# RenderKit/embree

Hardware: NVIDIA H100
Metric: Mrays/s incoherent diffuse-bounce, 10M-triangle scene (higher is better)
Workload: dtype f32

## Files before the change

### embree_b200/csrc/rtcore_shim.cpp

```cpp
#include <cuda_runtime.h>
#include <math.h>
#include <stdio.h>
#include <stdlib.h>
#include <string.h>

#include <algorithm>
#include <atomic>
#include <map>
#include <mutex>
#include <stdexcept>
#include <string>
#include <unordered_map>
#include <vector>

#include "../../include/embree4_b200.h"
#include "interp.cuh"
#include "rtk_device.h"

namespace {

struct ApiError {
  RTCError code;
  std::string msg;
};
// ... 567 lines not shown
void commit_scene(SceneImpl* s) {
  std::lock_guard<std::mutex> lk(s->commitMutex);
  std::vector<GeometryImpl*> geoms;
  {
    std::lock_guard<std::mutex> lg(s->geomMutex);
    if (!s->isModified()) return;
    geoms = s->geoms;
  }
  for (GeometryImpl* g : geoms)
    if (g && g->enabled && g->state == GeomState::MODIFIED) fail(RTC_ERROR_INVALID_OPERATION, "geometry not committed");
  if (s->progFn && !s->progFn(s->progPtr, 0.0)) fail(RTC_ERROR_CANCELLED, "progress monitor forced termination");
  s->dev->use();
  release_buffers(s->deviceBuffers);
  release_buffers(s->residentBuffers);
  s->residentCurves.clear();
  s->free_interp();
  const TwoLevelChoice twoLevel = choose_two_level(s, geoms);
  if (twoLevel.chosen) commit_two_level(s, geoms);
  else commit_single(s, geoms, twoLevel.possible);
}

struct ThreadCtx {
  int gpu = -1;
  cudaStream_t stream = nullptr;
  static constexpr size_t kStagingBytes = 16384;
  char* staging = nullptr;
  ~ThreadCtx() {
    if (staging) cudaFreeHost(staging);
    if (stream) cudaStreamDestroy(stream);
  }
  void ensure(int g) {
    if (gpu == g && stream) return;
    if (staging) { cudaFreeHost(staging); staging = nullptr; }
    if (stream) { cudaStreamDestroy(stream); stream = nullptr; }
    cudaSetDevice(g);
    cuda_check(cudaStreamCreateWithFlags(&stream, cudaStreamNonBlocking), "cudaStreamCreate");
    cuda_check(cudaHostAlloc(reinterpret_cast<void**>(&staging), kStagingBytes, cudaHostAllocMapped), "cudaHostAlloc");
    gpu = g;
  }
};
thread_local ThreadCtx t_ctx;

struct QueryArgs {
  uint32_t instID = RTC_INVALID_GEOMETRY_ID, instPrimID = RTC_INVALID_GEOMETRY_ID;
  RTCFilterFunctionN filter = nullptr;
  bool enforce = false;
  RTCRayQueryContext* ctx = nullptr;
};
template <typename Args>
QueryArgs read_args(const Args* a) {
  QueryArgs q;
  if (!a) return q;
  q.filter = a->filter;
  q.enforce = (a->flags & RTC_RAY_QUERY_FLAG_INVOKE_ARGUMENT_FILTER) != 0;
  q.ctx = a->context;
  if (a->context) { q.instID = a->context->instID[0]; q.instPrimID = a->context->instPrimID[0]; }
  return q;
}

bool filters_apply(SceneImpl* s, const QueryArgs& q, int occluded) {
  if (!q.filter && g_filterGeoms.load(std::memory_order_relaxed) == 0) return false;
  auto applies = [&](const GeometryImpl* g) {
    if (occluded ? g->occludedFilter != nullptr : g->intersectFilter != nullptr) return true;
    return q.filter && (q.enforce || g->argFilterEnabled);
  };
  std::lock_guard<std::mutex> lg(s->geomMutex);
  for (GeometryImpl* g : s->geoms) {
    if (!g || !g->enabled) continue;
    if (g->type != RTC_GEOMETRY_TYPE_INSTANCE) { if (applies(g)) return true; continue; }
    if (!g->instScene) continue;
    std::lock_guard<std::mutex> lc(g->instScene->geomMutex);
    for (GeometryImpl* cg : g->instScene->geoms)
      if (cg && cg->enabled && cg->type != RTC_GEOMETRY_TYPE_INSTANCE && applies(cg)) return true;
  }
  return false;
}

rtk::TraceParams make_params(SceneImpl* s, void* rays, const int* valid, unsigned long long n, uint32_t instID,
                             uint32_t instPrimID) {
  rtk::TraceParams p;
  p.nodes = s->gpu.nodes; p.tris = s->gpu.tris; p.root_valid = s->gpu.root_valid; p.robust = s->gpu.robust;
  p.descs = s->gpu.general ? s->gpu.d_descs : nullptr;
  p.curves = s->gpu.curves;
  p.top_nodes = s->gpu.levels.size() > 3 ? s->gpu.levels[3] : s->gpu.num_nodes;
  p.rays = rays; p.valid = valid; p.n = n; p.instID = instID; p.instPrimID = instPrimID;
  p.stat = s->statCounters ? s->gpu.d_stat : nullptr;
  return p;
}

void require_committed(SceneImpl* s) {
  if (!s->everCommitted) fail(RTC_ERROR_INVALID_OPERATION, "scene not committed");
}

void trace_one(SceneImpl* s, void* rec, size_t recBytes, const int* valid, int K, int occluded, uint32_t instID,
               uint32_t instPrimID) {
  require_committed(s);
  if (!s->gpu.root_valid) return;
  t_ctx.ensure(s->dev->gpu);
  cudaSetDevice(s->dev->gpu);
  memcpy(t_ctx.staging, rec, recBytes);
  int* sv = reinterpret_cast<int*>(t_ctx.staging + 1408);
  if (K > 1) memcpy(sv, valid, 4 * K);
  rtk::TraceParams p = make_params(s, t_ctx.staging, K > 1 ? sv : nullptr, (unsigned long long)K, instID, instPrimID);
  cuda_check((cudaError_t)rtk::launch_trace(p, occluded, K, t_ctx.stream), "trace launch");
  cuda_check(cudaStreamSynchronize(t_ctx.stream), "trace");
  memcpy(rec, t_ctx.staging, recBytes);
}

void trace_device(SceneImpl* s, void* d_rays, const int* d_valid, int K, size_t M, int occluded, uint32_t instID,
                  uint32_t instPrimID, cudaStream_t st, bool timeit, void* compact_out = nullptr) {
  require_committed(s);
  if (!s->gpu.root_valid || M == 0) return;
  cudaSetDevice(s->dev->gpu);
  rtk::TraceParams p = make_params(s, d_rays, d_valid, (unsigned long long)M * K, instID, instPrimID);
  p.compact_out = compact_out;
  if (timeit) {
    if (!s->ev0) { cudaEventCreate(&s->ev0); cudaEventCreate(&s->ev1); }
    cudaEventRecord(s->ev0, st);
  }
  cuda_check((cudaError_t)rtk::launch_trace(p, occluded, K, st), "trace launch");
  if (timeit) cudaEventRecord(s->ev1, st);
}

void trace_gather(SceneImpl* s, void* d_rays, size_t M, uint32_t instID, uint32_t instPrimID, cudaStream_t st, void* compact_out) {
  require_committed(s);
  if (M == 0) return;
  if (reinterpret_cast<uintptr_t>(compact_out) & 31) fail(RTC_ERROR_INVALID_ARGUMENT, "compact_out must be 32-byte aligned (one sector per record)");
  cudaSetDevice(s->dev->gpu);
  if (!s->ev0) { cudaEventCreate(&s->ev0); cudaEventCreate(&s->ev1); }
  cudaEventRecord(s->ev0, st);
  rtk::TraceParams p = make_params(s, d_rays, nullptr, (unsigned long long)M, instID, instPrimID);
  p.compact_out = compact_out;
  if (rtk::tuning().gather_mode == 1) {
    static thread_local struct Stage { int gpu = -1; void* p = nullptr; size_t cap = 0; ~Stage() { if (p) cudaFree(p); } } t_stage;
    if (t_stage.gpu != s->dev->gpu || t_stage.cap < M * 32) {
      if (t_stage.p) { cudaSetDevice(t_stage.gpu); cudaFree(t_stage.p); cudaSetDevice(s->dev->gpu); }
      t_stage.p = nullptr; t_stage.cap = 0; t_stage.gpu = s->dev->gpu;
      cuda_check(cudaMalloc(&t_stage.p, M * 32), "cudaMalloc(gather staging)");
      t_stage.cap = M * 32;
    }
    p.stage = t_stage.p;
  }
  cuda_check((cudaError_t)rtk::launch_trace(p, 0, 1, st), "trace launch");
  cudaEventRecord(s->ev1, st);
}

static int g_host_chunk_log2 = 20, g_host_streams = 3;
static int g_host_d2h_partial = 0;

struct HostPipe {
  int gpu = -1;
  static constexpr int kStreams = 6;
  cudaStream_t st[kStreams] = {};
  char* buf[kStreams] = {};
  int* vbuf[kStreams] = {};
  size_t cap = 0, vcap = 0;
  ~HostPipe() { reset(); }
  void reset() {
    for (int i = 0; i < kStreams; ++i) {
      if (buf[i]) cudaFree(buf[i]);
      if (vbuf[i]) cudaFree(vbuf[i]);
      if (st[i]) cudaStreamDestroy(st[i]);
      buf[i] = nullptr; vbuf[i] = nullptr; st[i] = nullptr;
    }
    cap = vcap = 0; gpu = -1;
  }
  void ensure(int g, size_t bytes, size_t vbytes) {
// ... 850 lines not shown
  scene_layout(g, &lay);
  s->dev->use();
  if (nodes && lay.num_nodes) cuda_check(cudaMemcpy(nodes, g.nodes, (size_t)lay.num_nodes * sizeof(rtk::Node8), cudaMemcpyDeviceToHost), "copy nodes");
  if (records && lay.num_records) cuda_check(cudaMemcpy(records, g.tris, (size_t)lay.num_records * sizeof(rtk::TriRec), cudaMemcpyDeviceToHost), "copy records");
  if (descs && lay.num_descs) {
    std::vector<rtk::GeomDesc> d(lay.num_descs);
    cuda_check(cudaMemcpy(d.data(), g.d_descs, d.size() * sizeof(rtk::GeomDesc), cudaMemcpyDeviceToHost), "copy descriptors");
    unsigned first = 0;
    for (size_t i = 0; i < d.size(); ++i) {
      RTCB200DescInfo& o = descs[i];
      o.geomID = d[i].geomID; o.instID = d[i].instID; o.kind = d[i].kind; o.first = first; o.count = d[i].ntris;
      o.is_quad = d[i].is_quad; o.tess = d[i].tess; o.basis = d[i].basis; o.hermite = d[i].hermite;
      memcpy(o.xfm, d[i].xfm, sizeof o.xfm);
      first += d[i].ntris;
    }
  }
  if (levels) for (unsigned l = 0; l < lay.num_levels; ++l) levels[l] = g.levels[l];
  if (subs)
    for (unsigned i = 0; i < lay.num_subs; ++i) {
      subs[4 * i] = g.sub_node_off[i]; subs[4 * i + 1] = g.sub_tri_off[i];
      subs[4 * i + 2] = g.sub_nodes[i]; subs[4 * i + 3] = g.sub_tris[i];
    }
  SCENE_END
}
void rtcb200SetSceneStatCounters(RTCScene sc, int enable) { SCENE_BEGIN(sc) S(sc)->statCounters = enable != 0; SCENE_END }
void rtcb200ResetSceneStatCounters(RTCScene sc) { SCENE_BEGIN(sc) if (S(sc)->gpu.d_stat) { S(sc)->dev->use(); cuda_check(cudaMemset(S(sc)->gpu.d_stat, 0, 24), "reset stat counters"); } SCENE_END }
unsigned long long rtcb200GetLaunchCount(void) { return rtk::launch_count(); }

void* rtcb200PeerAlloc(RTCDevice h, size_t bytes) {
  API_BEGIN
  VERIFY_HANDLE(h);
  D(h)->use();
  void* p = nullptr;
  cuda_check(cudaMalloc(&p, bytes ? bytes : 16), "cudaMalloc(peer buffer)");
  return p;
  API_END(D(h))
  return nullptr;
}
void rtcb200PeerFree(RTCDevice h, void* p) { API_BEGIN VERIFY_HANDLE(h); D(h)->use(); if (p) cuda_check(cudaFree(p), "cudaFree(peer buffer)"); API_END(D(h)) }
int rtcb200PeerExport(RTCDevice h, void* p, unsigned char handle[64]) {
  API_BEGIN
  VERIFY_HANDLE(h); VERIFY_HANDLE(p); VERIFY_HANDLE(handle);
  D(h)->use();
  static_assert(sizeof(cudaIpcMemHandle_t) == 64, "IPC handle size");
  cudaIpcMemHandle_t ih;
  cuda_check(cudaIpcGetMemHandle(&ih, p), "cudaIpcGetMemHandle");
  memcpy(handle, &ih, 64);
  return 0;
  API_END(D(h))
  return -1;
}
void* rtcb200PeerImport(RTCDevice h, const unsigned char handle[64]) {
  API_BEGIN
  VERIFY_HANDLE(h); VERIFY_HANDLE(handle);
  D(h)->use();
  cudaIpcMemHandle_t ih;
  memcpy(&ih, handle, 64);
  void* p = nullptr;
  cuda_check(cudaIpcOpenMemHandle(&p, ih, cudaIpcMemLazyEnablePeerAccess), "cudaIpcOpenMemHandle");
  return p;
  API_END(D(h))
  return nullptr;
}
void rtcb200PeerCopy(RTCDevice h, void* dst, const void* src, size_t bytes) {
  API_BEGIN VERIFY_HANDLE(h); D(h)->use(); cuda_check(cudaMemcpy(dst, src, bytes, cudaMemcpyDefault), "cudaMemcpy(peer buffer)"); API_END(D(h))
}
void rtcb200PeerClose(RTCDevice h, void* p) { API_BEGIN VERIFY_HANDLE(h); D(h)->use(); if (p) cuda_check(cudaIpcCloseMemHandle(p), "cudaIpcCloseMemHandle"); API_END(D(h)) }
int rtcb200SetTuning(const char* key, int value) {
  if (!key) return -1;
  rtk::Tuning& t = rtk::tuning();
  if (!strcmp(key, "collapse_policy")) t.collapse_policy = value;
  else if (!strcmp(key, "refill_min")) t.refill_min = value;
  else if (!strcmp(key, "sah_small")) t.sah_small = value;
  else if (!strcmp(key, "c_node")) t.c_node = value;
  else if (!strcmp(key, "c_tri")) t.c_tri = value;
  else if (!strcmp(key, "tri_batch_min")) t.tri_batch_min = value;
  else if (!strcmp(key, "tri_wait_max")) t.tri_wait_max = value;
  else if (!strcmp(key, "curve_batch_min")) t.curve_batch_min = value;
  else if (!strcmp(key, "curve_wait_max")) t.curve_wait_max = value;
  else if (!strcmp(key, "blocks_per_sm")) t.blocks_per_sm = value;
  else if (!strcmp(key, "curve_blocks_per_sm")) t.curve_blocks_per_sm = value;
  else if (!strcmp(key, "point_batch_min")) t.point_batch_min = value;
  else if (!strcmp(key, "point_wait_max")) t.point_wait_max = value;
  else if (!strcmp(key, "use_tma")) t.use_tma = value;
  else if (!strcmp(key, "tri_spread")) t.tri_spread = value != 0;
  else if (!strcmp(key, "tri_spread_occluded")) t.tri_spread_occluded = value != 0;
  else if (!strcmp(key, "gather_mode") && value >= 0 && value <= 1) t.gather_mode = value;
  else if (!strcmp(key, "host_d2h_partial")) g_host_d2h_partial = value != 0;
  else if (!strcmp(key, "host_chunk_log2") && value >= 10 && value <= 26) g_host_chunk_log2 = value;
  else if (!strcmp(key, "host_streams") && value >= 1 && value <= HostPipe::kStreams) g_host_streams = value;
  else return -1;
  return 0;
}
double rtcb200GetLastTraceMs(RTCScene sc) {
  SCENE_BEGIN(sc)
  SceneImpl* s = S(sc);
  if (!s->ev0) return -1.0;
  s->dev->use();
  cuda_check(cudaEventSynchronize(s->ev1), "event sync");
  float ms = 0;
  cuda_check(cudaEventElapsedTime(&ms, s->ev0, s->ev1), "event elapsed");
  return ms;
  SCENE_END
  return -1.0;
}

static void load_transform(RTCFormat format, const float* x, float out[12]) {
  switch ((int)format) {
    case 0x9134: { const float m[12] = {x[0], x[4], x[8], x[1], x[5], x[9], x[2], x[6], x[10], x[3], x[7], x[11]}; memcpy(out, m, sizeof m); break; }
    case 0x9234: memcpy(out, x, 12 * sizeof(float)); break;
    case 0x9244: { const float m[12] = {x[0], x[1], x[2], x[4], x[5], x[6], x[8], x[9], x[10], x[12], x[13], x[14]}; memcpy(out, m, sizeof m); break; }
    default: fail(RTC_ERROR_INVALID_OPERATION, "invalid matrix format");
  }
}
static void store_transform(const float m[12], RTCFormat format, float* x) {
  switch ((int)format) {
    case 0x9134: { const float o[12] = {m[0], m[3], m[6], m[9], m[1], m[4], m[7], m[10], m[2], m[5], m[8], m[11]}; memcpy(x, o, sizeof o); break; }
    case 0x9234: memcpy(x, m, 12 * sizeof(float)); break;
    case 0x9244: { const float o[16] = {m[0], m[1], m[2], 0, m[3], m[4], m[5], 0, m[6], m[7], m[8], 0, m[9], m[10], m[11], 1}; memcpy(x, o, sizeof o); break; }
    default: fail(RTC_ERROR_INVALID_OPERATION, "invalid matrix format");
  }
}
void rtcSetGeometryInstancedScene(RTCGeometry g, RTCScene scene) {
  GEOM_BEGIN(g)
  VERIFY_HANDLE(scene);
  if (G(g)->type != RTC_GEOMETRY_TYPE_INSTANCE) fail(RTC_ERROR_INVALID_OPERATION, "operation not supported for this geometry");
  if (G(g)->dev != S(scene)->dev) fail(RTC_ERROR_INVALID_ARGUMENT, "inputs are from different devices");
  S(scene)->retain();
  if (G(g)->instScene) G(g)->instScene->release();
  G(g)->instScene = S(scene);
  G(g)->update();
  GEOM_END
}
void rtcSetGeometryTransform(RTCGeometry g, unsigned int timeStep, enum RTCFormat format, const void* xfm) {
  GEOM_BEGIN(g)
  VERIFY_HANDLE(xfm);
  if (G(g)->type != RTC_GEOMETRY_TYPE_INSTANCE) fail(RTC_ERROR_INVALID_OPERATION, "operation not supported for this geometry");
  if (timeStep != 0) fail(RTC_ERROR_INVALID_OPERATION, "invalid timestep");
  load_transform(format, static_cast<const float*>(xfm), G(g)->xfm);
  G(g)->update_world2local();
  G(g)->update();
  GEOM_END
}
void rtcGetGeometryTransform(RTCGeometry g, float, enum RTCFormat format, void* xfm) {
  GEOM_BEGIN(g)
  VERIFY_HANDLE(xfm);
  store_transform(G(g)->xfm, format, static_cast<float*>(xfm));
  GEOM_END
}
void rtcGetGeometryTransformEx(RTCGeometry g, unsigned int, float time, enum RTCFormat format, void* xfm) { rtcGetGeometryTransform(g, time, format, xfm); }
void rtcGetGeometryTransformFromScene(RTCScene s, unsigned int id, float time, enum RTCFormat format, void* xfm) {
  SCENE_BEGIN(s)
  if (id >= S(s)->geoms.size() || !S(s)->geoms[id]) fail(RTC_ERROR_INVALID_ARGUMENT, "invalid geometry ID");
  rtcGetGeometryTransform(reinterpret_cast<RTCGeometry>(S(s)->geoms[id]), time, format, xfm);
  SCENE_END
}
void rtcGetGeometryTransformFromTraversable(RTCTraversable t, unsigned int id, float time, enum RTCFormat format, void* xfm) {
  rtcGetGeometryTransformFromScene(reinterpret_cast<RTCScene>(t), id, time, format, xfm);
}

void* rtcGetGeometryBufferDataDevice(RTCGeometry g, enum RTCBufferType type, unsigned int slot) { return rtcGetGeometryBufferData(g, type, slot); }
void rtcSetSharedGeometryBufferHostDevice(RTCGeometry g, enum RTCBufferType type, unsigned int slot, enum RTCFormat format, const void* ptr,
                                          const void* , size_t off, size_t stride, size_t num) {
  rtcSetSharedGeometryBuffer(g, type, slot, format, ptr, off, stride, num);
}
void rtcSetNewGeometryBufferHostDevice(RTCGeometry g, enum RTCBufferType type, unsigned int slot, enum RTCFormat format, size_t stride,
                                       size_t num, void** ptr, void** dptr) {
// ... 81 lines not shown
```

### embree_b200/csrc/rtk_device.h

```cpp
#pragma once
#include <cuda_runtime.h>
#include <stddef.h>
#include <stdint.h>

#include <vector>

#include "rt_core.cuh"

namespace rtk {

enum PrimKind : uint32_t {
  PRIM_TRIANGLE = 0,
  PRIM_ROUND_LINEAR = 1,
  PRIM_FLAT_LINEAR = 2,
  PRIM_FLAT_CUBIC = 3,
  PRIM_ROUND_CUBIC = 4,
  PRIM_SPHERE = 5,
  PRIM_DISC = 6,
  PRIM_ORIENTED_DISC = 7,
};
RT_HD constexpr bool curve_record(uint32_t kind) { return kind >= PRIM_ROUND_LINEAR && kind <= PRIM_ROUND_CUBIC; }
RT_HD constexpr bool point_record(uint32_t kind) { return kind >= PRIM_SPHERE; }

struct GeomDesc {
// ... 2 lines not shown
  uint64_t vstride, istride;
  uint32_t nverts, ntris;
  uint32_t geomID, mask;
  uint32_t has_xfm = 0, instID = 0xFFFFFFFFu, inst_mask = 0xFFFFFFFFu, skip_bounds = 0;
  uint32_t is_quad = 0;
  uint32_t kind = PRIM_TRIANGLE;
  const uint8_t* flags = nullptr;
  uint32_t basis = 0, tess = 4, hermite = 0;
  const float* basis_tab = nullptr;
  const uint8_t* tangents = nullptr;
  uint64_t tstride = 0;
  float xfm[12] = {1, 0, 0, 0, 1, 0, 0, 0, 1, 0, 0, 0};
  float w2l[12] = {1, 0, 0, 0, 1, 0, 0, 0, 1, 0, 0, 0};
};

#if defined(__CUDACC__)
__device__ __forceinline__ void load_cubic_cp(const GeomDesc& g, uint32_t vid, CurveVtx cp[4]) {
  if (g.hermite) {
    const float4 p0 = __ldg(reinterpret_cast<const float4*>(g.verts + (size_t)vid * g.vstride));
    const float4 p1 = __ldg(reinterpret_cast<const float4*>(g.verts + (size_t)(vid + 1) * g.vstride));
    const float4 t0 = __ldg(reinterpret_cast<const float4*>(g.tangents + (size_t)vid * g.tstride));
    const float4 t1 = __ldg(reinterpret_cast<const float4*>(g.tangents + (size_t)(vid + 1) * g.tstride));
    const float k = 1.0f / 3.0f;
    cp[0] = CurveVtx{p0.x, p0.y, p0.z, p0.w};
    cp[1] = CurveVtx{fma_rn(k, t0.x, p0.x), fma_rn(k, t0.y, p0.y), fma_rn(k, t0.z, p0.z), fma_rn(k, t0.w, p0.w)};
    cp[2] = CurveVtx{fma_rn(-k, t1.x, p1.x), fma_rn(-k, t1.y, p1.y), fma_rn(-k, t1.z, p1.z), fma_rn(-k, t1.w, p1.w)};
    cp[3] = CurveVtx{p1.x, p1.y, p1.z, p1.w};
    return;
  }
#pragma unroll
  for (int k = 0; k < 4; ++k) {
    const float4 q = __ldg(reinterpret_cast<const float4*>(g.verts + (size_t)(vid + k) * g.vstride));
    cp[k] = CurveVtx{q.x, q.y, q.z, q.w};
  }
}
#endif

enum BuilderKind : uint32_t { BUILDER_LBVH = 0, BUILDER_SAH = 1 };

struct SceneGPU {
  int device = 0;
  Node8* nodes = nullptr;
  TriRec* tris = nullptr;
  uint32_t num_nodes = 0, num_tris = 0;
  uint32_t root_valid = 0;
  int robust = 0;
  int general = 0;
  int curves = 0;
  GeomDesc* d_descs = nullptr;
  uint32_t num_descs = 0;
  float bounds[6] = {0, 0, 0, 0, 0, 0};
  float api_bounds[6] = {0, 0, 0, 0, 0, 0};
  double build_ms = 0, sah_cost = 0;
  uint32_t builder = 0, max_depth = 0;
  unsigned long long* d_stat = nullptr;
  size_t node_capacity = 0, tri_capacity = 0;
  uint32_t* tri_src = nullptr;
  uint32_t total_prims = 0;
  std::vector<uint32_t> levels;
  std::vector<uint32_t> sub_node_off, sub_tri_off, sub_nodes, sub_tris;
  std::vector<Node8> sub_root;
  std::vector<const void*> sub_id;
  uint32_t top_cap = 0;
  bool is_sub = false;
};

int assemble_scene(SceneGPU& top, SceneGPU* const* subs, int nsubs, const uint8_t* dirty, cudaStream_t stream, char* errmsg);

int build_scene(SceneGPU& s, const GeomDesc* geoms, int ngeoms, BuilderKind kind, cudaStream_t stream, char* errmsg);
int refit_scene(SceneGPU& s, const GeomDesc* geoms, int ngeoms, cudaStream_t stream, char* errmsg);
void free_scene(SceneGPU& s);

struct TraceParams {
  const Node8* nodes;
  const TriRec* tris;
  uint32_t root_valid;
  void* rays;
  const int* valid;
  unsigned long long n;
  uint32_t instID, instPrimID;
  unsigned long long* stat;
  void* compact_out = nullptr;
  void* stage = nullptr;
  int tri_batch_min = 8, tri_wait_max = 4, refill_min = 4, use_prefetch = 1;
  const GeomDesc* descs = nullptr;
  int curves = 0;
  uint32_t top_nodes = 0;
  int robust = 0;
  const uint32_t* excl_off = nullptr;
  const uint32_t* excl_idx = nullptr;
  uint32_t* win = nullptr;
};
int launch_trace(const TraceParams& p, int occluded, int K, cudaStream_t stream);

struct InterpEntry {
  uint32_t kind = 0;
  uint32_t basis = 0;
  uint32_t nprims = 0;
  uint32_t sub = 0;
  const uint8_t* idx = nullptr;
  const uint8_t* data = nullptr;
  const uint8_t* tang = nullptr;
  uint64_t istride = 0, dstride = 0, tstride = 0;
  uint64_t nelems = 0, ntang = 0;
};
struct InterpParams {
  const void* hits;
  unsigned long long M;
  const InterpEntry* table;
  uint32_t nentries;
  uint32_t valueCount;
  float* out[6];
};
int launch_interpolate(const InterpParams& p, cudaStream_t stream);

struct Tuning {
  int collapse_policy = 3;
  int c_node = 100, c_tri = 50;
  int tri_batch_min = 8;
  int tri_wait_max = 4;
  int curve_batch_min = 32, curve_wait_max = 24;
  int point_batch_min = 24, point_wait_max = 16;
  int blocks_per_sm = 8;
  int curve_blocks_per_sm = 6;
  int use_tma = 1;
  int refill_min = 4;
  int gather_mode = 1;
  int tri_spread = 1;
  int tri_spread_occluded = 1;
  int sah_small = 4;
};
Tuning& tuning();

void set_pool_keep_bytes(unsigned long long bytes);
unsigned long long launch_count();
void count_launch(unsigned n = 1);

}
```

### embree_b200/csrc/trace.cu

```cuda
#include <stdio.h>

#include "rtk_device.h"

namespace rtk {

__device__ __forceinline__ void ldg256(const void* p, uint32_t* d) {
  asm volatile("ld.global.nc.v4.b32 {%0,%1,%2,%3}, [%8];\n\t"
               "ld.global.nc.v4.b32 {%4,%5,%6,%7}, [%8+16];"
               : "=r"(d[0]), "=r"(d[1]), "=r"(d[2]), "=r"(d[3]), "=r"(d[4]), "=r"(d[5]), "=r"(d[6]), "=r"(d[7])
               : "l"(p));
}
__device__ __forceinline__ void load_node(const Node8* __restrict__ nodes, uint32_t node_index, NodeW& nw) {
  const char* np = reinterpret_cast<const char*>(nodes) + (size_t)node_index * sizeof(Node8);
  ldg256(np, nw.w); ldg256(np + 32, nw.w + 8); ldg256(np + 64, nw.w + 16);
}

template <int K, bool OCCLUDED>
struct RayIO;

template <bool OCCLUDED>
struct RayIO<1, OCCLUDED> {
  static constexpr int kStride = OCCLUDED ? 48 : 96;
  static constexpr int kRayBytes = kStride;
  static __device__ __forceinline__ void load(const char* base, unsigned long long i, Ray& r) {
    const float4* src = reinterpret_cast<const float4*>(base + i * kStride);
    const float4 a = src[0], b = src[1], c = src[2];
    r.ox = a.x; r.oy = a.y; r.oz = a.z; r.tnear = a.w;
    r.dx = b.x; r.dy = b.y; r.dz = b.z; r.time = b.w;
    r.tfar = c.x; r.mask = __float_as_uint(c.y); r.id = __float_as_uint(c.z); r.flags = __float_as_uint(c.w);
  }
  static __device__ __forceinline__ void store_tfar(const TraceParams& p, unsigned long long i, float tfar) {
    *reinterpret_cast<float*>(static_cast<char*>(p.rays) + i * kStride + 32) = tfar;
  }
  static __device__ __forceinline__ void store_hit(const TraceParams& p, unsigned long long i, const Hit& h, uint32_t instID, uint32_t instPrimID) {
    char* rec = static_cast<char*>(p.rays) + i * kStride;
    *reinterpret_cast<float*>(rec + 32) = h.t;
    float4 a, b;
    a.x = h.ngx; a.y = h.ngy; a.z = h.ngz; a.w = h.u;
    b.x = h.v; b.y = __uint_as_float(h.primID); b.z = __uint_as_float(h.geomID); b.w = __uint_as_float(instID);
    *reinterpret_cast<float4*>(rec + 48) = a;
    *reinterpret_cast<float4*>(rec + 64) = b;
    *reinterpret_cast<uint32_t*>(rec + 80) = instPrimID;
  }
};

template <int K, bool OCCLUDED>
struct RayIO {
  static constexpr int kPacket = (OCCLUDED ? 12 : 21) * 4 * K;
  static constexpr int kRayBytes = (OCCLUDED ? 12 : 21) * 4;
  static __device__ __forceinline__ char* field(const TraceParams& p, unsigned long long i, int f) {
    return static_cast<char*>(p.rays) + (i / K) * kPacket + ((size_t)f * K + (i % K)) * 4;
  }
  static __device__ __forceinline__ const char* cfield(const char* base, unsigned long long i, int f) {
    return base + (i / K) * kPacket + ((size_t)f * K + (i % K)) * 4;
  }
  static __device__ __forceinline__ void load(const char* base, unsigned long long i, Ray& r) {
    r.ox = *reinterpret_cast<const float*>(cfield(base, i, 0)); r.oy = *reinterpret_cast<const float*>(cfield(base, i, 1));
    r.oz = *reinterpret_cast<const float*>(cfield(base, i, 2)); r.tnear = *reinterpret_cast<const float*>(cfield(base, i, 3));
    r.dx = *reinterpret_cast<const float*>(cfield(base, i, 4)); r.dy = *reinterpret_cast<const float*>(cfield(base, i, 5));
    r.dz = *reinterpret_cast<const float*>(cfield(base, i, 6)); r.time = *reinterpret_cast<const float*>(cfield(base, i, 7));
    r.tfar = *reinterpret_cast<const float*>(cfield(base, i, 8)); r.mask = *reinterpret_cast<const uint32_t*>(cfield(base, i, 9));
    r.id = 0; r.flags = 0;
  }
  static __device__ __forceinline__ void store_tfar(const TraceParams& p, unsigned long long i, float tfar) {
    *reinterpret_cast<float*>(field(p, i, 8)) = tfar;
  }
  static __device__ __forceinline__ void store_hit(const TraceParams& p, unsigned long long i, const Hit& h, uint32_t instID, uint32_t instPrimID) {
    *reinterpret_cast<float*>(field(p, i, 8)) = h.t;
    *reinterpret_cast<float*>(field(p, i, 12)) = h.ngx; *reinterpret_cast<float*>(field(p, i, 13)) = h.ngy;
    *reinterpret_cast<float*>(field(p, i, 14)) = h.ngz; *reinterpret_cast<float*>(field(p, i, 15)) = h.u;
    *reinterpret_cast<float*>(field(p, i, 16)) = h.v; *reinterpret_cast<uint32_t*>(field(p, i, 17)) = h.primID;
    *reinterpret_cast<uint32_t*>(field(p, i, 18)) = h.geomID; *reinterpret_cast<uint32_t*>(field(p, i, 19)) = instID;
    *reinterpret_cast<uint32_t*>(field(p, i, 20)) = instPrimID;
  }
};

__device__ __forceinline__ float rcp_safe_fast(float d) {
  const float x = fabsf(d) < kMinRcpInput ? kMinRcpInput : d;
  const float r = __frcp_rn(x);
  return r;
}

__device__ __forceinline__ void to_object_space(const GeomDesc& d, Ray& r) {
  const float ox = r.ox, oy = r.oy, oz = r.oz, dx = r.dx, dy = r.dy, dz = r.dz;
  r.ox = fma_rn(ox, d.w2l[0], fma_rn(oy, d.w2l[3], fma_rn(oz, d.w2l[6], d.w2l[9])));
  r.oy = fma_rn(ox, d.w2l[1], fma_rn(oy, d.w2l[4], fma_rn(oz, d.w2l[7], d.w2l[10])));
  r.oz = fma_rn(ox, d.w2l[2], fma_rn(oy, d.w2l[5], fma_rn(oz, d.w2l[8], d.w2l[11])));
  r.dx = fma_rn(dx, d.w2l[0], fma_rn(dy, d.w2l[3], mul_rn(dz, d.w2l[6])));
  r.dy = fma_rn(dx, d.w2l[1], fma_rn(dy, d.w2l[4], mul_rn(dz, d.w2l[7])));
  r.dz = fma_rn(dx, d.w2l[2], fma_rn(dy, d.w2l[5], mul_rn(dz, d.w2l[8])));
}

__device__ __noinline__ bool round_record_test(const GeomDesc& d, const Ray& r, float tfar, uint32_t vid, int lane, CurveHit& h) {
  CurveVtx cp[4];
  load_cubic_cp(d, vid, cp);
  return round_cubic_test(r.ox, r.oy, r.oz, r.dx, r.dy, r.dz, r.tnear, tfar, cp, d.basis, h, lane);
}
__device__ __noinline__ bool curve_record_test(const GeomDesc& d, const Ray& r, float tfar, const uint4& a, const uint4& b, const uint4& c, CurveHit& h) {
  if (d.kind >= PRIM_SPHERE)
    return point_test(r.ox, r.oy, r.oz, r.dx, r.dy, r.dz, r.tnear, tfar, __uint_as_float(a.x), __uint_as_float(a.y), __uint_as_float(a.z),
                      __uint_as_float(c.x), __uint_as_float(b.x), __uint_as_float(b.y), __uint_as_float(b.z), (int)(d.kind - PRIM_SPHERE), h);
  if (d.kind == PRIM_ROUND_CUBIC) return round_record_test(d, r, tfar, c.z, (int)c.x, h);
  if (d.kind == PRIM_FLAT_CUBIC) {
    CurveVtx cp[4];
    load_cubic_cp(d, c.z, cp);
    return flat_cubic_test(r.ox, r.oy, r.oz, r.dx, r.dy, r.dz, r.tnear, tfar, cp, d.basis, (int)d.tess, d.basis_tab, h, (int)c.x);
  }
  const CurveVtx v0{__uint_as_float(a.x), __uint_as_float(a.y), __uint_as_float(a.z), __uint_as_float(c.x)};
  const CurveVtx v1{__uint_as_float(b.x), __uint_as_float(b.y), __uint_as_float(b.z), __uint_as_float(c.y)};
  if (d.kind == PRIM_FLAT_LINEAR)
    return flat_curve_test(r.ox, r.oy, r.oz, r.dx, r.dy, r.dz, r.tnear, tfar, v0, v1, h);
  const uint32_t vid = c.z & 0x3FFFFFFFu;
  const bool hasL = (c.z >> 30) & 1u, hasR = (c.z >> 31) & 1u;
  CurveVtx vL = v0, vR = v1;
  if (hasL) { const float4 q = __ldg(reinterpret_cast<const float4*>(d.verts + (size_t)(vid - 1) * d.vstride)); vL = CurveVtx{q.x, q.y, q.z, q.w}; }
  if (hasR) { const float4 q = __ldg(reinterpret_cast<const float4*>(d.verts + (size_t)(vid + 2) * d.vstride)); vR = CurveVtx{q.x, q.y, q.z, q.w}; }
  return curve_test(r.ox, r.oy, r.oz, r.dx, r.dy, r.dz, r.tnear, tfar, v0, v1, hasL, vL, hasR, vR, h);
}

__device__ __forceinline__ void store_256(void* dst, float a0, float a1, float a2, float a3, float a4, float a5, float a6, float a7) {
  asm volatile("st.global.v4.f32 [%0], {%1, %2, %3, %4};\n\t"
               "st.global.v4.f32 [%0+16], {%5, %6, %7, %8};" ::"l"(dst), "f"(a0), "f"(a1), "f"(a2), "f"(a3), "f"(a4),
               "f"(a5), "f"(a6), "f"(a7)
               : "memory");
}

constexpr int TRACE_THREADS = 128;
constexpr int TRACE_WARPS = TRACE_THREADS / 32;

__device__ __forceinline__ void tma_prefetch_l2(const void* src, uint32_t bytes) {
  asm volatile("cp.async.bulk.prefetch.L2.global [%0], %1;" ::"l"(src), "r"(bytes) : "memory");
}

#ifndef RTK_MIN_BLOCKS
#define RTK_MIN_BLOCKS 8
#endif
#ifndef RTK_SMEM_STACK
#define RTK_SMEM_STACK 8
#endif
#ifndef RTK_TOP_SMEM
#define RTK_TOP_SMEM 0
#endif
#ifndef RTK_LANE_SMEM
#define RTK_LANE_SMEM 1
#endif
#ifndef RTK_CHILD_PREFETCH
#define RTK_CHILD_PREFETCH 0
#endif
#ifndef RTK_TRI2
#define RTK_TRI2 1
#endif

template <int K, bool OCCLUDED, bool STATS, bool ROBUST, int GENERAL, int GATHER = 0, bool SPREAD = false, bool FILTER = false>
__global__ void __launch_bounds__(TRACE_THREADS, RTK_MIN_BLOCKS) trace_kernel(const TraceParams p) {
  const bool USE_TMA = p.use_prefetch != 0;
  using IO = RayIO<K, OCCLUDED>;
  const unsigned FULL = 0xFFFFFFFFu;
  const int lane = threadIdx.x & 31;
  const unsigned lt_mask = (1u << lane) - 1u;
  const uint32_t warp_id = blockIdx.x * TRACE_WARPS + (threadIdx.x >> 5);
  const uint32_t num_warps = gridDim.x * TRACE_WARPS;
  const uint32_t n = (uint32_t)p.n;
  const Node8* __restrict__ nodes = p.nodes;
  const uint4* __restrict__ tris = reinterpret_cast<const uint4*>(p.tris);
  const int tri_batch_min = p.tri_batch_min, tri_wait_max = p.tri_wait_max, refill_min = p.refill_min;

  enum : uint32_t { EMPTY = 0, TRACING = 1, DONE = 2 };
  uint32_t state = EMPTY;
  Ray r;
  float idx = 0, idy = 0, idz = 0, tfar_tri = 0;
  uint32_t oct = 0;
#if RTK_LANE_SMEM
  __shared__ uint32_t s_lane[GENERAL == 2 ? 12 : 9][TRACE_THREADS];
#define hit_u (reinterpret_cast<float*>(s_lane[0])[threadIdx.x])
#define hit_v (reinterpret_cast<float*>(s_lane[1])[threadIdx.x])
#define hit_tri (s_lane[2][threadIdx.x])
#define ray_index (s_lane[3][threadIdx.x])
#define RAY_DX(t) (reinterpret_cast<float*>(s_lane[4])[t])
#define RAY_DY(t) (reinterpret_cast<float*>(s_lane[5])[t])
#define RAY_DZ(t) (reinterpret_cast<float*>(s_lane[6])[t])
#define RAY_MASK(t) (s_lane[7][t])
#define RAY_TFAR(t) (reinterpret_cast<float*>(s_lane[8])[t])
#else
  float hit_u = 0, hit_v = 0;
  uint32_t hit_tri = 0;
  uint32_t ray_index = 0;
#error "RTK_LANE_SMEM=0 is no longer supported"
#endif
  auto full_ray = [&]() -> Ray {
    Ray q = r;
    q.dx = RAY_DX(threadIdx.x); q.dy = RAY_DY(threadIdx.x); q.dz = RAY_DZ(threadIdx.x);
    q.mask = RAY_MASK(threadIdx.x); q.tfar = RAY_TFAR(threadIdx.x);
    return q;
  };
  bool found = false;
  uint32_t ngx = 0, ngy = 0, tgx = 0, tgy = 0;
  uint32_t top_x = 0, top_y = 0;
  __shared__ uint2 s_stack[RTK_SMEM_STACK > 0 ? RTK_SMEM_STACK * TRACE_THREADS : 1];
  uint2 stack[kStackSize];
  int sp = 0;
  auto push_entry = [&](uint32_t x, uint32_t y) {
    if (sp < RTK_SMEM_STACK) s_stack[sp * TRACE_THREADS + threadIdx.x] = make_uint2(x, y);
    else stack[sp - RTK_SMEM_STACK] = make_uint2(x, y);
    ++sp;
  };
  auto pop_entry = [&]() -> uint2 {
    --sp;
    return sp < RTK_SMEM_STACK ? s_stack[sp * TRACE_THREADS + threadIdx.x] : stack[sp - RTK_SMEM_STACK];
  };
  int blk = -1;
  uint32_t blk_first = 0, blk_count = 0, consumed = 0;
  bool warp_done = false;
  int tri_wait = 0;
  unsigned long long st_rays = 0, st_nodes = 0, st_tris = 0;
  __shared__ uint32_t s_slot[GATHER == 2 ? TRACE_WARPS : 1][4];
  constexpr uint32_t kNoBlock = 0xFFFFFFFFu;
  if (GATHER == 2) {
    if (lane < 4) s_slot[threadIdx.x >> 5][lane] = (lane & 1) ? 0u : kNoBlock;
    __syncwarp();
  }

  auto block_first = [&](int b) -> unsigned long long { return ((unsigned long long)b * num_warps + warp_id) * 32ull; };
  auto prefetch = [&](int b) {
    const unsigned long long first = block_first(b);
    if (first >= n) return;
    const uint32_t cnt = (n - first) < 32u ? (uint32_t)(n - first) : 32u;
    tma_prefetch_l2(static_cast<const char*>(p.rays) + first * IO::kRayBytes, cnt * IO::kRayBytes);
  };
  if (USE_TMA && lane == 0) { prefetch(0); prefetch(1); }
#if RTK_TOP_SMEM > 0
  __shared__ alignas(128) uint32_t s_top[RTK_TOP_SMEM * 24];
  __shared__ alignas(8) unsigned long long s_top_bar;
  const uint32_t top_nodes = p.top_nodes < (uint32_t)RTK_TOP_SMEM ? p.top_nodes : (uint32_t)RTK_TOP_SMEM;
  if (top_nodes) {
    const uint32_t bar = (uint32_t)__cvta_generic_to_shared(&s_top_bar), dst = (uint32_t)__cvta_generic_to_shared(s_top);
    if (threadIdx.x == 0) {
      asm volatile("mbarrier.init.shared::cta.b64 [%0], 1;" ::"r"(bar));
      asm volatile("fence.mbarrier_init.release.cluster;" ::: "memory");
      asm volatile("mbarrier.arrive.expect_tx.shared::cta.b64 _, [%0], %1;" ::"r"(bar), "r"(top_nodes * 96u) : "memory");
      asm volatile("cp.async.bulk.shared::cluster.global.mbarrier::complete_tx::bytes [%0], [%1], %2, [%3];" ::"r"(dst), "l"(p.nodes),
                   "r"(top_nodes * 96u), "r"(bar)
                   : "memory");
    }
    __syncthreads();
    uint32_t done = 0;
    while (!done)
      asm volatile("{ .reg .pred q; mbarrier.try_wait.parity.shared::cta.b64 q, [%1], 0; selp.u32 %0, 1, 0, q; }" : "=r"(done) : "r"(bar) : "memory");
  }
// ... 143 lines not shown
        state = EMPTY;
      }
      if (GATHER == 2) {
        const unsigned have0 = ss[1] | __reduce_or_sync(FULL, slot == 0 ? 1u << (ray_index & 31u) : 0u);
        const unsigned have1 = ss[3] | __reduce_or_sync(FULL, slot == 1 ? 1u << (ray_index & 31u) : 0u);
        auto full_mask = [&](uint32_t first) -> unsigned { return (n - first) >= 32u ? 0xFFFFFFFFu : ((1u << (n - first)) - 1u); };
        const bool done0 = first0 != kNoBlock && have0 == full_mask(first0), done1 = first1 != kNoBlock && have1 == full_mask(first1);
        if (done0) flush_block(first0, have0);
        if (done1) flush_block(first1, have1);
        __syncwarp();
        if (lane == 0) { ss[0] = done0 ? kNoBlock : first0; ss[1] = done0 ? 0u : have0; ss[2] = done1 ? kNoBlock : first1; ss[3] = done1 ? 0u : have1; }
        __syncwarp();
      }
      if (!warp_done) {
        if (consumed == blk_count) {
          if (USE_TMA && lane == 0) prefetch(blk + 3);
          ++blk;
          const unsigned long long first = block_first(blk);
          if (first >= n) { warp_done = true; blk_count = 0; consumed = 0; }
          else {
            blk_first = (uint32_t)first;
            blk_count = (n - blk_first) < 32u ? (n - blk_first) : 32u;
            consumed = 0;
            if (GATHER == 2) {
              uint32_t* ss = s_slot[threadIdx.x >> 5];
              const uint32_t f0 = ss[0], h0 = ss[1], f1 = ss[2], h1 = ss[3];
              int use = f0 == kNoBlock ? 0 : (f1 == kNoBlock ? 1 : (f0 < f1 ? 0 : 1));
              if (f0 != kNoBlock && f1 != kNoBlock) flush_block(use == 0 ? f0 : f1, use == 0 ? h0 : h1);
              __syncwarp();
              if (lane == 0) { ss[2 * use] = blk_first; ss[2 * use + 1] = 0u; }
              __syncwarp();
            }
          }
        }
        if (!warp_done) {
          const uint32_t avail = blk_count - consumed;
          const uint32_t rank = __popc(idle & lt_mask);
          if (state == EMPTY && rank < avail) {
            ray_index = blk_first + consumed + rank;
            bool valid = true;
            if (K > 1) valid = (p.valid == nullptr) || (p.valid[ray_index] == -1);
            if (valid) {
              IO::load(static_cast<const char*>(p.rays), ray_index, r);
              if (STATS) ++st_rays;
              found = false;
              sp = 0; top_y = 0; tgx = 0; tgy = 0;
              const bool go = p.root_valid && !(OCCLUDED && r.tfar < 0.0f);
              RAY_DX(threadIdx.x) = r.dx; RAY_DY(threadIdx.x) = r.dy; RAY_DZ(threadIdx.x) = r.dz;
              RAY_MASK(threadIdx.x) = r.mask; RAY_TFAR(threadIdx.x) = r.tfar;
              idx = rcp_safe_fast(r.dx); idy = rcp_safe_fast(r.dy); idz = rcp_safe_fast(r.dz);
              oct = (idx < 0.0f ? 1u : 0u) | (idy < 0.0f ? 2u : 0u) | (idz < 0.0f ? 4u : 0u);
              tfar_tri = r.tfar;
              ngx = 0; ngy = go ? 0x80000000u : 0u;
              state = go ? TRACING : DONE;
            }
          }
          const uint32_t want = __popc(idle);
          consumed += want < avail ? want : avail;
        }
      }
      if (!__any_sync(FULL, state == TRACING)) {
        if (warp_done && !__any_sync(FULL, state == DONE)) break;
        continue;
      }
    }
    const bool tracing = state == TRACING;
    if (tracing && tgy == 0 && (ngy & 0xFF000000u)) {
      const int bit = 31 - __clz((int)ngy);
      ngy &= ~(1u << bit);
      if (ngy & 0xFF000000u) {
        if (top_y) push_entry(top_x, top_y);
        top_x = ngx; top_y = ngy;
      }
      const uint32_t slot = ((uint32_t)(bit - 24)) ^ (7u - oct);
      const uint32_t node_index = ngx + (uint32_t)__popc(ngy & 0xFFu & ((1u << slot) - 1u));
      NodeW nw;
#if RTK_TOP_SMEM > 0
      if (node_index < top_nodes) {
        const uint4* sp4 = reinterpret_cast<const uint4*>(s_top + node_index * 24);
#pragma unroll
        for (int k = 0; k < 6; ++k) { const uint4 q = sp4[k]; nw.w[4 * k] = q.x; nw.w[4 * k + 1] = q.y; nw.w[4 * k + 2] = q.z; nw.w[4 * k + 3] = q.w; }
      } else
#endif
      load_node(nodes, node_index, nw);
      if (STATS) ++st_nodes;
      const uint32_t hm = node_hitmask(nw.w, r.ox, r.oy, r.oz, idx, idy, idz, (oct & 1u) != 0, (oct & 2u) != 0, (oct & 4u) != 0,
                                       fmaxf(r.tnear, 0.0f), fmaxf(tfar_tri, 0.0f), 7u - oct);
      ngx = nw.w[4];
      ngy = (hm & 0xFF000000u) | (nw.w[3] >> 24);
      tgx = nw.w[5];
      tgy = hm & 0x00FFFFFFu;
#if RTK_CHILD_PREFETCH == 1
      {
        const uint32_t pend = ngy >> 24;
        if (pend & (pend - 1u)) tma_prefetch_l2(reinterpret_cast<const char*>(nodes) + (size_t)ngx * sizeof(Node8), (uint32_t)__popc(ngy & 0xFFu) * (uint32_t)sizeof(Node8));
      }
#elif RTK_CHILD_PREFETCH == 2
      {
        const uint32_t pend = ngy >> 24;
        if (pend & (pend - 1u)) {
          const int b2 = 31 - __clz((int)(ngy & ~(1u << (31 - __clz((int)ngy)))));
          const uint32_t slot2 = ((uint32_t)(b2 - 24)) ^ (7u - oct);
          const char* a2 = reinterpret_cast<const char*>(nodes) + (size_t)(ngx + (uint32_t)__popc(ngy & 0xFFu & ((1u << slot2) - 1u))) * sizeof(Node8);
          asm volatile("prefetch.global.L2 [%0];" ::"l"(a2));
          asm volatile("prefetch.global.L2 [%0];" ::"l"(a2 + 64));
        }
      }
#endif
    }
    const unsigned tri_lanes = __ballot_sync(FULL, tracing && tgy != 0);
    const unsigned node_lanes = __ballot_sync(FULL, tracing && tgy == 0 && (ngy & 0xFF000000u));
    if (tri_lanes && (__popc(tri_lanes) >= tri_batch_min || node_lanes == 0 || ++tri_wait >= tri_wait_max)) {
      tri_wait = 0;
      if (SPREAD) {
        __shared__ uint32_t s_tri[TRACE_WARPS][32];
        __shared__ uint32_t s_owner[TRACE_WARPS][32];
        __shared__ unsigned long long s_best[TRACE_WARPS][32];
        const int wi = threadIdx.x >> 5;
        const bool isT = tracing && tgy != 0;
        const int cnt = isT ? __popc(tgy) : 0;
        int incl = cnt;
#pragma unroll
        for (int o = 1; o < 32; o <<= 1) { const int v = __shfl_up_sync(FULL, incl, o); if (lane >= o) incl += v; }
        int slot = incl - cnt;
        const int total = min(__shfl_sync(FULL, incl, 31), 32);
        s_best[wi][lane] = ~0ull;
        while (isT && tgy != 0 && slot < 32) {
          const int tb = 31 - __clz((int)tgy);
          tgy &= ~(1u << tb);
          s_tri[wi][slot] = tgx + (uint32_t)tb;
          s_owner[wi][slot] = (uint32_t)lane;
          ++slot;
        }
        __syncwarp();
        const bool work = lane < total;
        const uint32_t ti = work ? s_tri[wi][lane] : 0u;
        const int owner = work ? (int)s_owner[wi][lane] : lane;
        Ray lr;
        lr.ox = __shfl_sync(FULL, r.ox, owner); lr.oy = __shfl_sync(FULL, r.oy, owner); lr.oz = __shfl_sync(FULL, r.oz, owner);
        const int ot = (threadIdx.x & ~31) + owner;
        lr.dx = RAY_DX(ot); lr.dy = RAY_DY(ot); lr.dz = RAY_DZ(ot);
        lr.tnear = __shfl_sync(FULL, r.tnear, owner);
        const float o_tfar = RAY_TFAR(ot);
        const float o_best = __shfl_sync(FULL, tfar_tri, owner);
        const uint32_t o_mask = RAY_MASK(ot);
        float w_u = 0.0f, w_v = 0.0f;
        unsigned long long key = ~0ull;
        if (work) {
          const uint4* tp = tris + (size_t)ti * 3;
          const uint4 a = __ldg(tp), b = __ldg(tp + 1), c = __ldg(tp + 2);
          if (STATS) ++st_tris;
          TriHit th;
          if ((c.w & o_mask) != 0 &&
              tri_test(lr, o_tfar, __uint_as_float(a.x), __uint_as_float(a.y), __uint_as_float(a.z), __uint_as_float(b.x),
                       __uint_as_float(b.y), __uint_as_float(b.z), __uint_as_float(c.x), __uint_as_float(c.y), __uint_as_float(c.z), th)) {
            if (OCCLUDED) {
              s_best[wi][owner] = 0ull;
            } else {
            const float rcpAbsDen = 1.0f / th.absDen;
            const float t = th.T * rcpAbsDen;
            if (t <= o_best) {
              w_u = th.U * rcpAbsDen; w_v = th.V * rcpAbsDen;
              uint32_t tb32 = __float_as_uint(t);
              tb32 ^= (tb32 >> 31) ? 0xFFFFFFFFu : 0x80000000u;
              key = ((unsigned long long)tb32 << 32) | (uint32_t)(31 - lane);
              atomicMin(&s_best[wi][owner], key);
            }
// ... 26 lines not shown
          const int tb2 = two ? 31 - __clz((int)tgy) : tb;
          const uint32_t ti2 = tgx + (uint32_t)tb2;
          const uint4* tp2 = tris + (size_t)ti2 * 3;
          uint4 a2, b2, c2;
          if (two) { a2 = __ldg(tp2); b2 = __ldg(tp2 + 1); c2 = __ldg(tp2 + 2); }
          test_tri(ti, a, b, c);
          if (two && tgy != 0) {
            tgy &= ~(1u << tb2);
            if (STATS) ++st_tris;
            test_tri(ti2, a2, b2, c2);
          }
        } else {
          test_tri(ti, a, b, c);
        }
      }
    }
    if (tracing && tgy == 0 && (ngy & 0xFF000000u) == 0) {
      if (top_y) { ngx = top_x; ngy = top_y; top_y = 0; }
      else if (sp > 0) { const uint2 e = pop_entry(); ngx = e.x; ngy = e.y; }
      else state = DONE;
    }
  }
  if (GATHER == 2) {
    const uint32_t* ss = s_slot[threadIdx.x >> 5];
    if (ss[0] != kNoBlock && ss[1]) flush_block(ss[0], ss[1]);
    if (ss[2] != kNoBlock && ss[3]) flush_block(ss[2], ss[3]);
  }
  if (STATS) {
#pragma unroll
    for (int o = 16; o > 0; o >>= 1) {
      st_rays += __shfl_xor_sync(FULL, st_rays, o);
      st_nodes += __shfl_xor_sync(FULL, st_nodes, o);
      st_tris += __shfl_xor_sync(FULL, st_tris, o);
    }
    if (lane == 0) { atomicAdd(&p.stat[0], st_rays); atomicAdd(&p.stat[1], st_nodes); atomicAdd(&p.stat[2], st_tris); }
  }
}

#if RTK_LANE_SMEM
#undef hit_u
#undef hit_v
#undef hit_tri
#undef ray_index
#undef RAY_DX
#undef RAY_DY
#undef RAY_DZ
#undef RAY_MASK
#undef RAY_TFAR
#endif

static int g_num_sms = 0;
static Tuning g_tuning;
Tuning& tuning() { return g_tuning; }

template <int K, bool OCCLUDED>
static int launch_k(TraceParams p, cudaStream_t st) {
  if (p.n == 0) return 0;
  if (p.n > 0x40000000ull) {
    const unsigned long long chunk = 0x40000000ull;
    for (unsigned long long first = 0; first < p.n; first += chunk) {
      TraceParams q = p;
      q.n = (p.n - first) < chunk ? (p.n - first) : chunk;
      q.rays = static_cast<char*>(p.rays) + first * RayIO<K, OCCLUDED>::kRayBytes;
      if (p.valid) q.valid = p.valid + first;
      if (p.compact_out) q.compact_out = static_cast<char*>(p.compact_out) + first * 32;
      if (p.stage) q.stage = static_cast<char*>(p.stage) + first * 32;
      const int r = launch_k<K, OCCLUDED>(q, st);
      if (r != 0) return r;
    }
    return 0;
  }
  if (!g_num_sms) {
    int dev = 0;
    cudaGetDevice(&dev);
    cudaDeviceGetAttribute(&g_num_sms, cudaDevAttrMultiProcessorCount, dev);
    if (g_num_sms <= 0) g_num_sms = 132;
  }
  p.tri_batch_min = p.curves == 2 ? g_tuning.curve_batch_min : p.curves ? g_tuning.point_batch_min : g_tuning.tri_batch_min;
  p.tri_wait_max = p.curves == 2 ? g_tuning.curve_wait_max : p.curves ? g_tuning.point_wait_max : g_tuning.tri_wait_max;
  p.refill_min = g_tuning.refill_min;
  const unsigned long long need = (p.n + TRACE_THREADS - 1) / TRACE_THREADS;
  const unsigned long long cap = (unsigned long long)g_num_sms * (p.curves == 2 ? g_tuning.curve_blocks_per_sm : g_tuning.blocks_per_sm);
  const unsigned blocks = (unsigned)(need < cap ? need : cap);
  p.use_prefetch = (p.n >= 1024 && g_tuning.use_tma) ? 1 : 0;
  constexpr bool CLOSEST = !OCCLUDED;
  constexpr bool CAN_GATHER = (K == 1 && CLOSEST);
  const int variant = (p.stat ? 4 : 0) | (p.robust ? 2 : 0) | (p.descs ? 1 : 0);
  if (p.excl_off) {
    if (!(K == 1 && CLOSEST) || !p.excl_idx || !p.win) return (int)cudaErrorInvalidValue;
    constexpr bool FI = (K == 1 && CLOSEST);
    const int g = !p.descs ? 0 : (p.curves ? 2 : 1);
    switch (g * 2 + (p.robust ? 1 : 0)) {
#define RTK_FILTER(RB, GE) trace_kernel<K, OCCLUDED, false, RB, GE, 0, false, FI><<<blocks, TRACE_THREADS, 0, st>>>(p); break
      case 0: RTK_FILTER(false, 0);
      case 1: RTK_FILTER(true, 0);
      case 2: RTK_FILTER(false, 1);
      case 3: RTK_FILTER(true, 1);
      case 4: RTK_FILTER(false, 2);
      case 5: RTK_FILTER(true, 2);
#undef RTK_FILTER
    }
    count_launch();
    return (int)cudaGetLastError();
  }
  if (p.descs && p.curves) {
    const int gmode = (CAN_GATHER && p.compact_out) ? ((g_tuning.gather_mode == 0 || !p.stage) ? 1 : 2) : 0;
    switch ((variant >> 1) + 4 * gmode) {
#define RTK_CURVE(ST, RB, GA) trace_kernel<K, OCCLUDED, ST, RB, 2, (CAN_GATHER ? GA : 0), false><<<blocks, TRACE_THREADS, 0, st>>>(p); break
#define RTK_CURVE4(GA)                         \
      case 4 * GA + 0: RTK_CURVE(false, false, GA); \
      case 4 * GA + 1: RTK_CURVE(false, true, GA);  \
      case 4 * GA + 2: RTK_CURVE(true, false, GA);  \
      case 4 * GA + 3: RTK_CURVE(true, true, GA);
      RTK_CURVE4(0)
      RTK_CURVE4(1)
      RTK_CURVE4(2)
#undef RTK_CURVE4
#undef RTK_CURVE
    }
    count_launch();
    return (int)cudaGetLastError();
  }
  const int gather = (CAN_GATHER && p.compact_out) ? ((g_tuning.gather_mode == 0 || !p.stage) ? 1 : 2) : 0;
  const bool spread = (CLOSEST ? g_tuning.tri_spread : g_tuning.tri_spread_occluded) && !p.robust && !p.descs;
  switch (variant + 8 * gather + (spread ? 32 : 0)) {
#define RTK_LAUNCH(ST, RB, IN, GA, SP) trace_kernel<K, OCCLUDED, ST, RB, (IN ? 1 : 0), (CAN_GATHER ? GA : 0), SP><<<blocks, TRACE_THREADS, 0, st>>>(p); break
#define RTK_LAUNCH8(GA)                                          \
    case 8 * GA + 0: RTK_LAUNCH(false, false, false, GA, false); \
    case 8 * GA + 1: RTK_LAUNCH(false, false, true, GA, false);  \
    case 8 * GA + 2: RTK_LAUNCH(false, true, false, GA, false);  \
    case 8 * GA + 3: RTK_LAUNCH(false, true, true, GA, false);   \
    case 8 * GA + 4: RTK_LAUNCH(true, false, false, GA, false);  \
    case 8 * GA + 5: RTK_LAUNCH(true, false, true, GA, false);   \
    case 8 * GA + 6: RTK_LAUNCH(true, true, false, GA, false);   \
    case 8 * GA + 7: RTK_LAUNCH(true, true, true, GA, false);    \
    case 32 + 8 * GA + 0: RTK_LAUNCH(false, false, false, GA, true); \
    case 32 + 8 * GA + 4: RTK_LAUNCH(true, false, false, GA, true);
    RTK_LAUNCH8(0)
    RTK_LAUNCH8(1)
    RTK_LAUNCH8(2)
#undef RTK_LAUNCH8
#undef RTK_LAUNCH
  }
  count_launch();
  return (int)cudaGetLastError();
}

int launch_trace(const TraceParams& p, int occluded, int K, cudaStream_t st) {
  switch (K) {
    case 1: return occluded ? launch_k<1, true>(p, st) : launch_k<1, false>(p, st);
    case 4: return occluded ? launch_k<4, true>(p, st) : launch_k<4, false>(p, st);
    case 8: return occluded ? launch_k<8, true>(p, st) : launch_k<8, false>(p, st);
    case 16: return occluded ? launch_k<16, true>(p, st) : launch_k<16, false>(p, st);
  }
  return (int)cudaErrorInvalidValue;
}

}
```

Baseline: 1283.

## Pin top BVH levels in L2 via cache policy, drop TMA prefetch for triangles

```diff
diff --git a/embree_b200/csrc/l2_cut.h b/embree_b200/csrc/l2_cut.h
--- /dev/null
+++ b/embree_b200/csrc/l2_cut.h
@@ -0,0 +1,16 @@
+#pragma once
+#include <stddef.h>
+#include <stdint.h>
+
+namespace rtk {
+
+inline uint32_t l2_node_cut(const uint32_t* levels, size_t nlevels, size_t node_bytes, size_t budget_bytes) {
+  uint32_t cut = 0;
+  for (size_t l = 0; l < nlevels; ++l) {
+    if ((size_t)levels[l] * node_bytes > budget_bytes) break;
+    cut = levels[l];
+  }
+  return cut;
+}
+
+}
diff --git a/embree_b200/csrc/rtcore_shim.cpp b/embree_b200/csrc/rtcore_shim.cpp
--- a/embree_b200/csrc/rtcore_shim.cpp
+++ b/embree_b200/csrc/rtcore_shim.cpp
@@ -673,7 +673,7 @@
   p.nodes = s->gpu.nodes; p.tris = s->gpu.tris; p.root_valid = s->gpu.root_valid; p.robust = s->gpu.robust;
   p.descs = s->gpu.general ? s->gpu.d_descs : nullptr;
   p.curves = s->gpu.curves;
-  p.top_nodes = s->gpu.levels.size() > 3 ? s->gpu.levels[3] : s->gpu.num_nodes;
+  p.top_nodes = rtk::node_l2_cut(s->gpu.levels, s->dev->gpu);
   p.rays = rays; p.valid = valid; p.n = n; p.instID = instID; p.instPrimID = instPrimID;
   p.stat = s->statCounters ? s->gpu.d_stat : nullptr;
   return p;
@@ -1690,7 +1690,6 @@
   else if (!strcmp(key, "curve_blocks_per_sm")) t.curve_blocks_per_sm = value;
   else if (!strcmp(key, "point_batch_min")) t.point_batch_min = value;
   else if (!strcmp(key, "point_wait_max")) t.point_wait_max = value;
-  else if (!strcmp(key, "use_tma")) t.use_tma = value;
   else if (!strcmp(key, "tri_spread")) t.tri_spread = value != 0;
   else if (!strcmp(key, "tri_spread_occluded")) t.tri_spread_occluded = value != 0;
   else if (!strcmp(key, "gather_mode") && value >= 0 && value <= 1) t.gather_mode = value;
diff --git a/embree_b200/csrc/rtk_device.h b/embree_b200/csrc/rtk_device.h
--- a/embree_b200/csrc/rtk_device.h
+++ b/embree_b200/csrc/rtk_device.h
@@ -108,7 +108,7 @@
   unsigned long long* stat;
   void* compact_out = nullptr;
   void* stage = nullptr;
-  int tri_batch_min = 8, tri_wait_max = 4, refill_min = 4, use_prefetch = 1;
+  int tri_batch_min = 8, tri_wait_max = 4, refill_min = 4, use_prefetch = 0;
   const GeomDesc* descs = nullptr;
   int curves = 0;
   uint32_t top_nodes = 0;
@@ -118,6 +118,7 @@
   uint32_t* win = nullptr;
 };
 int launch_trace(const TraceParams& p, int occluded, int K, cudaStream_t stream);
+uint32_t node_l2_cut(const std::vector<uint32_t>& levels, int device);
 
 struct InterpEntry {
   uint32_t kind = 0;
@@ -149,7 +150,6 @@
   int point_batch_min = 24, point_wait_max = 16;
   int blocks_per_sm = 8;
   int curve_blocks_per_sm = 6;
-  int use_tma = 1;
   int refill_min = 4;
   int gather_mode = 1;
   int tri_spread = 1;
diff --git a/embree_b200/csrc/trace.cu b/embree_b200/csrc/trace.cu
--- a/embree_b200/csrc/trace.cu
+++ b/embree_b200/csrc/trace.cu
@@ -1,18 +1,38 @@
 #include <stdio.h>
 
+#include "l2_cut.h"
 #include "rtk_device.h"
 
 namespace rtk {
 
+__device__ __forceinline__ void ldg256(const void* p, uint64_t pol, uint32_t* d) {
+  asm volatile("ld.global.nc.L2::cache_hint.v4.b32 {%0,%1,%2,%3}, [%8], %9;\n\t"
+               "ld.global.nc.L2::cache_hint.v4.b32 {%4,%5,%6,%7}, [%8+16], %9;"
+               : "=r"(d[0]), "=r"(d[1]), "=r"(d[2]), "=r"(d[3]), "=r"(d[4]), "=r"(d[5]), "=r"(d[6]), "=r"(d[7])
+               : "l"(p), "l"(pol));
+}
 __device__ __forceinline__ void ldg256(const void* p, uint32_t* d) {
   asm volatile("ld.global.nc.v4.b32 {%0,%1,%2,%3}, [%8];\n\t"
                "ld.global.nc.v4.b32 {%4,%5,%6,%7}, [%8+16];"
                : "=r"(d[0]), "=r"(d[1]), "=r"(d[2]), "=r"(d[3]), "=r"(d[4]), "=r"(d[5]), "=r"(d[6]), "=r"(d[7])
                : "l"(p));
 }
+__device__ __forceinline__ void load_node(const Node8* __restrict__ nodes, uint32_t node_index, uint64_t pol, NodeW& nw) {
+  const char* np = reinterpret_cast<const char*>(nodes) + (size_t)node_index * sizeof(Node8);
+  ldg256(np, pol, nw.w); ldg256(np + 32, pol, nw.w + 8); ldg256(np + 64, pol, nw.w + 16);
+}
 __device__ __forceinline__ void load_node(const Node8* __restrict__ nodes, uint32_t node_index, NodeW& nw) {
   const char* np = reinterpret_cast<const char*>(nodes) + (size_t)node_index * sizeof(Node8);
   ldg256(np, nw.w); ldg256(np + 32, nw.w + 8); ldg256(np + 64, nw.w + 16);
+}
+__device__ __forceinline__ uint64_t node_policy(const Node8* nodes, uint32_t cut) {
+  uint64_t pol;
+  if (cut)
+    asm("createpolicy.range.global.L2::evict_last.L2::evict_unchanged.b64 %0, [%1], %2, %3;"
+        : "=l"(pol) : "l"(nodes), "r"(cut * (uint32_t)sizeof(Node8)), "r"(0xFFFFFFFFu));
+  else
+    asm("createpolicy.fractional.L2::evict_normal.b64 %0, 1.0;" : "=l"(pol));
+  return pol;
 }
 
 template <int K, bool OCCLUDED>
@@ -164,6 +184,7 @@
   const Node8* __restrict__ nodes = p.nodes;
   const uint4* __restrict__ tris = reinterpret_cast<const uint4*>(p.tris);
   const int tri_batch_min = p.tri_batch_min, tri_wait_max = p.tri_wait_max, refill_min = p.refill_min;
+  const uint64_t node_pol = GENERAL == 2 ? 0ull : node_policy(nodes, p.top_nodes);
 
   enum : uint32_t { EMPTY = 0, TRACING = 1, DONE = 2 };
   uint32_t state = EMPTY;
@@ -473,7 +494,8 @@
         for (int k = 0; k < 6; ++k) { const uint4 q = sp4[k]; nw.w[4 * k] = q.x; nw.w[4 * k + 1] = q.y; nw.w[4 * k + 2] = q.z; nw.w[4 * k + 3] = q.w; }
       } else
 #endif
-      load_node(nodes, node_index, nw);
+      if (GENERAL == 2) load_node(nodes, node_index, nw);
+      else load_node(nodes, node_index, node_pol, nw);
       if (STATS) ++st_nodes;
       const uint32_t hm = node_hitmask(nw.w, r.ox, r.oy, r.oz, idx, idy, idz, (oct & 1u) != 0, (oct & 2u) != 0, (oct & 4u) != 0,
                                        fmaxf(r.tnear, 0.0f), fmaxf(tfar_tri, 0.0f), 7u - oct);
@@ -666,7 +688,7 @@
   const unsigned long long need = (p.n + TRACE_THREADS - 1) / TRACE_THREADS;
   const unsigned long long cap = (unsigned long long)g_num_sms * (p.curves == 2 ? g_tuning.curve_blocks_per_sm : g_tuning.blocks_per_sm);
   const unsigned blocks = (unsigned)(need < cap ? need : cap);
-  p.use_prefetch = (p.n >= 1024 && g_tuning.use_tma) ? 1 : 0;
+  p.use_prefetch = (p.n >= 1024 && p.curves) ? 1 : 0;
   constexpr bool CLOSEST = !OCCLUDED;
   constexpr bool CAN_GATHER = (K == 1 && CLOSEST);
   const int variant = (p.stat ? 4 : 0) | (p.robust ? 2 : 0) | (p.descs ? 1 : 0);
@@ -730,6 +752,16 @@
   return (int)cudaGetLastError();
 }
 
+uint32_t node_l2_cut(const std::vector<uint32_t>& levels, int device) {
+  static int l2_bytes[64] = {};
+  int& l2 = l2_bytes[device >= 0 && device < 64 ? device : 0];
+  if (!l2) {
+    cudaDeviceGetAttribute(&l2, cudaDevAttrL2CacheSize, device);
+    if (l2 <= 0) l2 = 50 << 20;
+  }
+  return l2_node_cut(levels.data(), levels.size(), sizeof(Node8), (size_t)l2 / 20);
+}
+
 int launch_trace(const TraceParams& p, int occluded, int K, cudaStream_t st) {
   switch (K) {
     case 1: return occluded ? launch_k<1, true>(p, st) : launch_k<1, false>(p, st);
```

Measured after the change: 1306 (median of 6 runs). 1.02x the previous value.
